# artpixls/ART

Hardware: AMD Instinct MI355X
Metric: megapixels/sec end-to-end (AMaZE+FTblockDN+tone), 45 MP Bayer (higher is better)
Workload: dtype f32; 1 GPU; AMaZE + getImage/matrix + ImProcFunctions::denoise (chroma noise-curve map, FTblockDN wavelet shrinkage luma 40 / chroma 15 / gamma 1.7 + DCT detail recovery 50) + exposure 0.3 EV + tone curve STD, 8192x5464 Bayer RGGB fp32, 1 frame per GPU per step (BASELINE configs[2]); frame=8192x5464, lanes_per_gpu=1, parallelism=frame-per-gpu x1, completion_records=1, completion_via=single process

## Files before the change

### art_amd/csrc/amaze_stream_core.h

```cpp
#pragma once

#ifdef AMZ_EMUL
#include <math.h>
#include <stdint.h>
#include <string.h>
#define AMZ_DEV static inline
typedef float *amz_lf;
typedef unsigned char *amz_lb;
typedef int *amz_li;
typedef unsigned short *amz_ls;
typedef char *amz_lc;
typedef const float *amz_gcf;
typedef float *amz_gf;
namespace amz {
static inline unsigned fc(unsigned filters, unsigned row, unsigned col) { return (filters >> (((((row) << 1) & 14u) + ((col) & 1u)) << 1)) & 3u; }
static inline float sse_min(float x, float y) { return x < y ? x : y; }
static inline float sse_max(float x, float y) { return x > y ? x : y; }
static inline float sqr(float x) { return x * x; }
static inline float intp(float a, float b, float c) { return a * b + (1.f - a) * c; }
static inline float median3(float a, float b, float c) { return sse_max(sse_min(a, b), sse_min(c, sse_max(a, b))); }
static inline float xdiv2f(float d) { int32_t i; memcpy(&i, &d, 4); if (i & 0x7FFFFFFF) i -= 1 << 23; memcpy(&d, &i, 4); return d; }
static inline float xdivf(float d, int n) { int32_t i; memcpy(&i, &d, 4); if (i & 0x7FFFFFFF) i -= n << 23; memcpy(&d, &i, 4); return d; }
static inline int ngroups(int start, int bound, int step) { return bound > start ? (bound - start + step - 1) / step : 0; }
static inline int imin(int a, int b) { return a < b ? a : b; }
// ... 298 lines not shown
        const float cl1 = cr[c - 1], cl2 = cr[c - 2], cr1 = cr[c + 1], cr2 = cr[c + 2];
        const float d0c = d0r[c], d1c = d1r[c];
        const float d0u2 = ROWR(D0, r - 2)[c], d0d2 = ROWR(D0, r + 2)[c], d1l2 = d1r[c - 2], d1r2 = d1r[c + 2];
        const float cru = cu1 * (d0u2 + d0c) / (d0u2 * (eps + cfav) + d0c * (eps + cu2));
        const float crd = cd1 * (d0d2 + d0c) / (d0d2 * (eps + cfav) + d0c * (eps + cd2));
        const float crl = cl1 * (d1l2 + d1c) / (d1l2 * (eps + cfav) + d1c * (eps + cl2));
        const float crr = cr1 * (d1r2 + d1c) / (d1r2 * (eps + cfav) + d1c * (eps + cr2));
        const float guha = cu1 + 0.5f * (cfav - cu2);
        const float gdha = cd1 + 0.5f * (cfav - cd2);
        const float glha = cl1 + 0.5f * (cfav - cl2);
        const float grha = cr1 + 0.5f * (cfav - cr2);
        float guar = fabsf(1.f - cru) < arthresh ? cfav * cru : guha;
        float gdar = fabsf(1.f - crd) < arthresh ? cfav * crd : gdha;
        float glar = fabsf(1.f - crl) < arthresh ? cfav * crl : glha;
        float grar = fabsf(1.f - crr) < arthresh ? cfav * crr : grha;
        const float d1l = d1r[c - 1], d1rr = d1r[c + 1], d0u = ROWR(D0, r - 1)[c], d0d = ROWR(D0, r + 1)[c];
        const float hwt = d1l / (d1l + d1rr);
        const float vwt = d0u / (d0d + d0u);
        const float Ginthha = intp(hwt, grha, glha);
        const float Gintvha = intp(vwt, gdha, guha);
        o_hcdalt = sgn * (Ginthha - cfav);
        o_vcdalt = sgn * (Gintvha - cfav);
        const bool clip = (cfav > a.clip_pt8) || (Gintvha > a.clip_pt8) || (Ginthha > a.clip_pt8);
        if (clip) { guar = guha; gdar = gdha; glar = glha; grar = grha; }
        o_vcd = clip ? o_vcdalt : sgn * (intp(vwt, gdar, guar) - cfav);
        o_hcd = clip ? o_hcdalt : sgn * (intp(hwt, grar, glar) - cfav);
        ROWW(DGV, r)[c] = sse_min(sqr(guha - gdha), sqr(guar - gdar));
        ROWW(DGH, r)[c] = sse_min(sqr(glha - grha), sqr(glar - grar));
        if (!is_green(a, r, c)) {
            amz_lf hv = ROWW(HVW, r);
            hv[c >> 1] = hwt;
            hv[TSH + (c >> 1)] = vwt;
        }
    }
    ROWW(HCA, r)[c] = o_hcdalt;
    ROWW(VCA, r)[c] = o_vcdalt;
    ROWW(VCD, r)[c] = o_vcd;
    ROWW(HCO, r)[c] = o_hcd;
}

AMZ_DEV float p3_hcd_pure(amz_lf ho, amz_lf ha, amz_lf cf, const TileArgs &a, int r, int c)
{
    const float sgn = is_green(a, r, c) ? -1.f : 1.f;
    float hcdv = ho[c];
    const float hv = var3(ho[c - 2], hcdv, ho[c + 2]);
    const float a0 = ha[c];
    const float hav = var3(ha[c - 2], a0, ha[c + 2]);
    hcdv = hav < hv ? a0 : hcdv;
    return bound_cd(hcdv, sgn, cf[c], cf[c - 1], cf[c + 1], a.clip_pt);
}
#ifdef AMZ_EMUL
#define AMZ_P3_COL(c) (c)
#else
#define AMZ_P3_COL(c) ((c) - 2)
#endif
AMZ_DEV void st_p3(amz_lf lds, const TileArgs &a, int r, int c_in)
{
    const int c = AMZ_P3_COL(c_in);
#ifdef AMZ_EMUL
    if (r < 4 || r >= a.rr1 - 4 || c >= TS) return;
#else
    if (r < 4 || r >= a.rr1 - 4) return;
#endif
    float nh = 0.f;
    const bool dom = c >= 4 && c < TS - 4;
    amz_lf ho = ROWR(HCO, r), ha = ROWR(HCA, r), cf = ROWR(CFA, r);
    const int idx = c - 4, k = idx & 3, g = idx >> 2;
#ifndef AMZ_EMUL
    float pure = 0.f;
    if (dom) pure = p3_hcd_pure(ho, ha, cf, a, r, c);
    const float left2 = __shfl_up(pure, 2);
    if (c < 0 || c >= TS) return;
#endif
    if (dom) {
        if (k >= 2) {
#ifdef AMZ_EMUL
            nh = p3_hcd_pure(ho, ha, cf, a, r, c);
#else
            nh = pure;
#endif
        } else {
#ifdef AMZ_EMUL
            const float hm2 = g > 0 ? p3_hcd_pure(ho, ha, cf, a, r, c - 2) : ho[c - 2];
#else
            const float hm2 = g > 0 ? left2 : ho[c - 2];
#endif
            const float sgn = is_green(a, r, c) ? -1.f : 1.f;
            float hcdv = ho[c];
            const float hv = var3(hm2, hcdv, ho[c + 2]);
            const float a0 = ha[c];
            const float hav = var3(ha[c - 2], a0, ha[c + 2]);
            hcdv = hav < hv ? a0 : hcdv;
            nh = bound_cd(hcdv, sgn, cf[c], cf[c - 1], cf[c + 1], a.clip_pt);
        }
        const float sgn = is_green(a, r, c) ? -1.f : 1.f;
        amz_lf vr = ROWR(VCD, r);
        const float n2 = ROWR(VCD, r - 2)[c];
        const float o0 = vr[c], o2 = ROWR(VCD, r + 2)[c];
        const float am2 = ROWR(VCA, r - 2)[c], a0 = ROWR(VCA, r)[c], a2 = ROWR(VCA, r + 2)[c];
        const float cm1 = ROWR(CFA, r - 1)[c], c0 = cf[c], cp1 = ROWR(CFA, r + 1)[c];
        float vcdv = o0;
        const float vv = var3(n2, vcdv, o2);
        const float vav = var3(am2, a0, a2);
        vcdv = vav < vv ? a0 : vcdv;
        const float nv = bound_cd(vcdv, sgn, c0, cm1, cp1, a.clip_pt);
        vr[c] = nv;
        const float cdq = sqr(nv - nh);
        ROWW(CDD, r)[c] = cdq;
        if (r == 19 && c >= 80 && c < 120) lds[NQA_OFF + (c - 80)] = cdq;
    }
    ROWW(HCN, r)[c] = nh;
}

AMZ_DEV int site_sel(const TileArgs &a, int r, int c) { return (c ^ row_par(a, r)) & 1; }

AMZ_DEV void st_p4(amz_lf lds, const TileArgs &a, int r, int c)
{
    if (c >= TS) return;
    const int sl = site_sel(a, r, c), rr = r + sl;
    if (rr < 6 || rr >= a.rr1 - 6) return;
    const int par = row_par(a, rr);
    if (c < 6 + par || c > 156 + par) return;
    amz_lf hn = SROWR(HCN, r, 0, sl), dh = SROWR(DGH, r, 0, sl);
    float tv = SROWR(VCD, r, 0, sl)[c];
    const float vu1 = SROWR(VCD, r, -1, sl)[c], vu2 = SROWR(VCD, r, -2, sl)[c], vu3 = SROWR(VCD, r, -3, sl)[c];
    const float vd1 = SROWR(VCD, r, +1, sl)[c], vd2 = SROWR(VCD, r, +2, sl)[c], vd3 = SROWR(VCD, r, +3, sl)[c];
    const float uave = tv + vu1 + vu2 + vu3;
    const float dave = tv + vd1 + vd2 + vd3;
    float Dvu = sqr(tv - uave) + sqr(vu1 - uave) + sqr(vu2 - uave) + sqr(vu3 - uave);
    float Dvd = sqr(tv - dave) + sqr(vd1 - dave) + sqr(vd2 - dave) + sqr(vd3 - dave);
    amz_lf hv = SROWR(HVW, r, 0, sl);
    const float hwt = hv[c >> 1], vwt = hv[TSH + (c >> 1)];
    const float vcd_c = tv;
    tv = hn[c];
#define COLZ(row, cc) ((cc) < TS ? (row)[cc] : 0.f)
    const float hl1 = hn[c - 1], hl2 = hn[c - 2], hl3 = hn[c - 3];
    const float hr1 = COLZ(hn, c + 1), hr2 = COLZ(hn, c + 2), hr3 = COLZ(hn, c + 3);
    const float lave = tv + (hl3 + hl2) + hl1;
    const float rave = tv + (hr1 + hr2) + hr3;
    float Dhl = sqr(tv - lave) + sqr(hl1 - lave) + sqr(hl2 - lave) + sqr(hl3 - lave);
    float Dhr = sqr(tv - rave) + sqr(hr1 - rave) + sqr(hr2 - rave) + sqr(hr3 - rave);
    const float vcdvar = epssq + intp(vwt, Dvd, Dvu);
    const float hcdvar = epssq + intp(hwt, Dhr, Dhl);
    Dvu = SROWR(DGV, r, -1, sl)[c] + SROWR(DGV, r, -2, sl)[c];
    Dvd = SROWR(DGV, r, +1, sl)[c] + SROWR(DGV, r, +2, sl)[c];
    Dhl = dh[c - 2] + dh[c - 1];
    Dhr = COLZ(dh, c + 1) + COLZ(dh, c + 2);
#undef COLZ
    const float vcdvar1 = epssq + SROWR(DGV, r, 0, sl)[c] + intp(vwt, Dvd, Dvu);
    const float hcdvar1 = epssq + dh[c] + intp(hwt, Dhr, Dhl);
    const float varwt = hcdvar / (vcdvar + hcdvar);
    const float diffwt = hcdvar1 / (vcdvar1 + hcdvar1);
    const bool dec = ((0.5f - varwt) * (0.5f - diffwt) > 0.f) && (fabsf(0.5f - diffwt) < fabsf(0.5f - varwt));
    SROWW(HVWT, r, 0, sl)[c >> 1] = dec ? varwt : diffwt;
    amz_lf vh = SROWW(VH, r, 0, sl);
    vh[c >> 1] = vcd_c;
    vh[TSH + (c >> 1)] = tv;
}

struct ThreadRegs { int bb[4]; int pos_p, pos_h, pos_stride2, pos_off4; };
AMZ_DEV void bb_reset(int *bb) { bb[0] = 1 << 30; bb[1] = 0; bb[2] = 1 << 30; bb[3] = 0; }
AMZ_DEV void bb_add(int *bb, int rr, int cc) { bb[0] = imin(bb[0], rr); bb[1] = imax(bb[1], rr); bb[2] = imin(bb[2], cc); bb[3] = imax(bb[3], cc); }
AMZ_DEV void bb_flush(amz_lf lds, int base, const int *bb)
{
    if (bb[1] == 0 && bb[3] == 0) return;
    amz_li red = (amz_li)(lds + RED_OFF) + base;
#ifdef AMZ_EMUL
    red[0] = imin(red[0], bb[0]); red[1] = imax(red[1], bb[1]); red[2] = imin(red[2], bb[2]); red[3] = imax(red[3], bb[3]);
#else
    __hip_atomic_fetch_min(&red[0], bb[0], __ATOMIC_RELAXED, __HIP_MEMORY_SCOPE_WORKGROUP);
    __hip_atomic_fetch_max(&red[1], bb[1], __ATOMIC_RELAXED, __HIP_MEMORY_SCOPE_WORKGROUP);
    __hip_atomic_fetch_min(&red[2], bb[2], __ATOMIC_RELAXED, __HIP_MEMORY_SCOPE_WORKGROUP);
    __hip_atomic_fetch_max(&red[3], bb[3], __ATOMIC_RELAXED, __HIP_MEMORY_SCOPE_WORKGROUP);
#endif
}

AMZ_DEV void pos_init(amz_lf lds, int c, ThreadRegs &rg)
{
    if (c >= POS_PAIRS) return;
    rg.pos_h = POSTAB.h[c]; rg.pos_stride2 = POSTAB.stride2[c]; rg.pos_off4 = POSTAB.off4[c];
    rg.pos_p = (rg.pos_h - POSTAB.j[c]) % rg.pos_h;
    ((amz_li)(lds + POS_OFF))[c] = rg.pos_off4 + rg.pos_p * rg.pos_stride2;
}
AMZ_DEV void pos_produce(amz_lf lds, int T, int c, ThreadRegs &rg)
{
    if (c >= POS_PAIRS) return;
    rg.pos_p = rg.pos_p + 1 == rg.pos_h ? 0 : rg.pos_p + 1;
    ((amz_li)(lds + POS_OFF + ((T + 1) & 1) * POS_PAIRS))[c] = rg.pos_off4 + rg.pos_p * rg.pos_stride2;
}

AMZ_DEV void st_p5(amz_lf lds, const TileArgs &a, int r, int c, ThreadRegs &rg)
{
    if (r + 1 < 6 || r >= a.rr1 - 6) return;
    if (c >= TS) {
        const int h = c - TS;
        if (h < 12) {
            const int sl = h >= 6, k = h % 6;
            if (r + sl < 6 || r + sl >= a.rr1 - 6) return;
            amz_lb nb = (amz_lb)SROWW(NYQ, r, 0, sl);
            nb[k < 3 ? k : 74 + k] = 0;
        }
        return;
    }
    const int sl = site_sel(a, r, c), rr = r + sl;
    if (rr < 6 || rr >= a.rr1 - 6) return;
    const int par = row_par(a, rr);
    if (c < 6 + par) return;
    amz_lb nb = (amz_lb)SROWW(NYQ, r, 0, sl);
    if (c >= TS - 6) { nb[c >> 1] = 0; return; }
    const float go0 = 0.14659727707323927f, go1 = 0.103592713382435f, go2 = 0.0732036125103057f, go3 = 0.0365543548389495f;
    const float nyqthresh = 0.5f;
    const float gg0 = nyqthresh * 0.07384411893421103f, gg1 = nyqthresh * 0.06207511968171489f, gg2 = nyqthresh * 0.0521818194747806f;
    const float gg3 = nyqthresh * 0.03687419286733595f, gg4 = nyqthresh * 0.03099732204057846f, gg5 = nyqthresh * 0.018413194161458882f;
    const int si = (c - 6 - par) >> 1;
    const bool vec = si < 4 * ngroups(6 + par, TS - 7, 8);
    amz_lf c0 = SROWR(CDD, r, 0, sl), cu1 = SROWR(CDD, r, -1, sl), cu2 = SROWR(CDD, r, -2, sl), cd1 = SROWR(CDD, r, +1, sl), cd2 = SROWR(CDD, r, +2, sl);
    amz_lf d0 = SROWR(DHV, r, 0, sl), du1 = SROWR(DHV, r, -1, sl), du2 = SROWR(DHV, r, -2, sl), dd1 = SROWR(DHV, r, +1, sl), dd2 = SROWR(DHV, r, +2, sl);
    const float gA = go0 * c0[c] +
                     go1 * (cu1[c - 1] + cu1[c + 1] + cd1[c - 1] + cd1[c + 1]) +
                     go2 * (cu2[c] + c0[c - 2] + c0[c + 2] + cd2[c]) +
                     go3 * (cu2[c - 2] + cu2[c + 2] + cd2[c - 2] + cd2[c + 2]);
    const float s1 = vec ? (du1[c] + d0[c - 1] + d0[c + 1] + dd1[c])
                         : (du1[c] + d0[c + 1] + d0[c - 1] + dd1[c]);
    const float gB = gg0 * d0[c] + gg1 * s1 +
                     gg2 * (du1[c - 1] + du1[c + 1] + dd1[c - 1] + dd1[c + 1]) +
                     gg3 * (du2[c] + d0[c - 2] + d0[c + 2] + dd2[c]) +
                     gg4 * (du2[c - 1] + du2[c + 1] + du1[c - 2] + du1[c + 2] +
                            dd1[c - 2] + dd1[c + 2] + dd2[c - 1] + dd2[c + 1]) +
                     gg5 * (du2[c - 2] + du2[c + 2] + dd2[c - 2] + dd2[c + 2]);
    const bool flag = gA - gB > 0.f;
    nb[c >> 1] = flag ? 1 : 0;
    if (flag) bb_add(rg.bb, rr, c);
}

AMZ_DEV void st_p7(amz_lf lds, const TileArgs &a, int r, int item)
{
    if (item >= 2 * TSH) return;
    const int sl = item >= TSH, rr = r + sl, b = item - (sl ? TSH : 0);
    if (rr < 2 || rr >= a.rr1 - 2) return;
    amz_lb out = (amz_lb)SROWW(NYQ2, r, 0, sl);
    if (rr < ny_r0(a) || rr >= ny_r1(a)) {
        out[b] = rr >= TS - 4 ? ((amz_lb)(lds + NQA_OFF))[(rr - (TS - 4)) * TSH + b] : 0;
        return;
    }
    amz_lb n0 = (amz_lb)SROWR(NYQ, r, 0, sl), nu1 = (amz_lb)SROWR(NYQ, r, -1, sl), nu2 = (amz_lb)SROWR(NYQ, r, -2, sl);
    amz_lb nd1 = (amz_lb)SROWR(NYQ, r, +1, sl), nd2 = (amz_lb)SROWR(NYQ, r, +2, sl);
    const int bl = b - 1, br = b + 1;
    const int t = (int)nu2[b] + (bl >= 0 ? (int)nu1[bl] : 0) + (int)nu1[b] + (bl >= 0 ? (int)n0[bl] : 0) +
                  (br < TSH ? (int)n0[br] : 0) + (bl >= 0 ? (int)nd1[bl] : 0) + (int)nd1[b] + (int)nd2[b];
    unsigned char val = n0[b];
    if (t > 4) val = 1;
    if (t < 4) val = 0;
    out[b] = val;
}

AMZ_DEV bool nyq_site(amz_lf lds, const TileArgs &a, int r, int c, int *prr)
{
    if (c >= TS) return false;
    const int sl = site_sel(a, r, c), rr = r + sl;
    *prr = rr;
    if (rr < ny_r0(a) || rr >= ny_r1(a) || c < ny_c0(a) + row_par(a, rr) || c >= ny_c1(a)) return false;
    return ((amz_lb)SROWR(NYQ2, r, 0, sl))[c >> 1] != 0;
}

struct P8Acc { float sumcfa, sumh, sumv, sumsqh, sumsqv, areawt; };
template <int A0, int A1>
AMZ_DEV void p8_accumulate(amz_lf lds, const TileArgs &a, int r, int sl, int cc, P8Acc &s)
{
    const int idx0 = (cc - 6) >> 1;
#pragma unroll
    for (int ai = A0; ai <= A1; ai += 2) {
        amz_lb nq = (amz_lb)SROWR(NYQ2, r, ai, sl);
        amz_lf cr = SROWR(CFA, r, ai, sl), cu = SROWR(CFA, r, ai - 1, sl), cd = SROWR(CFA, r, ai + 1, sl);
#pragma unroll
        for (int bj = 0; bj < 7; ++bj) {
            const bool f = nq[idx0 + bj] != 0;
            const int col = cc - 6 + 2 * bj;
            const float ct = cr[col], cl = cr[col - 1], cq = cr[col + 1], cn = cu[col], cs = cd[col];
            const float t1 = f ? ct : 0.f;
            const float t2 = f ? (cl + cq) : 0.f;
            const float t3 = f ? (cn + cs) : 0.f;
            const float t4 = f ? (sqr(ct - cl) + sqr(ct - cq)) : 0.f;
            const float t5 = f ? (sqr(ct - cn) + sqr(ct - cs)) : 0.f;
            s.sumcfa += t1;
            s.sumh += t2;
            s.sumv += t3;
            s.sumsqh += t4;
            s.sumsqv += t5;
            s.areawt += f ? 1.f : 0.f;
        }
    }
}
AMZ_DEV void p8_finish(amz_lf lds, const TileArgs &a, int r, int sl, int cc, const P8Acc &s, int *bb)
{
    const int rr = r + sl;
    const float sumh = s.sumcfa - xdiv2f(s.sumh);
    const float sumv = s.sumcfa - xdiv2f(s.sumv);
    const float areawt = xdiv2f(s.areawt);
    const float hcdvar = epssq + fabsf(areawt * s.sumsqh - sumh * sumh);
    const float vcdvar = epssq + fabsf(areawt * s.sumsqv - sumv * sumv);
    SROWR(HVWT, r, 0, sl)[cc >> 1] = hcdvar / (vcdvar + hcdvar);
    bb_add(bb, rr, cc);
}
struct P8Regs { P8Acc acc; int sl, cc; };
AMZ_DEV void p8_wave_a(amz_lf lds, const TileArgs &a, int t, int r, int lane, P8Regs &pr)
{
    amz_li red = (amz_li)(lds + RED_OFF);
    amz_ls list = (amz_ls)(lds + LIST_OFF + (t & 1) * LIST_INTS);
    const int n = red[16 + (t & 1)];
    pr.cc = -1;
    if (lane < n) {
        const int e = list[lane];
        pr.sl = (e >> 8) - r; pr.cc = e & 255;
        pr.acc = P8Acc{0.f, 0.f, 0.f, 0.f, 0.f, 0.f};
        p8_accumulate<-6, 0>(lds, a, r, pr.sl, pr.cc, pr.acc);
    }
}
AMZ_DEV void p8_wave_b(amz_lf lds, const TileArgs &a, int t, int r, int lane, P8Regs &pr, int *bb)
{
    amz_li red = (amz_li)(lds + RED_OFF);
    amz_ls list = (amz_ls)(lds + LIST_OFF + (t & 1) * LIST_INTS);
    const int n = red[16 + (t & 1)];
    if (pr.cc >= 0) {
        p8_accumulate<2, 6>(lds, a, r, pr.sl, pr.cc, pr.acc);
        p8_finish(lds, a, r, pr.sl, pr.cc, pr.acc, bb);
    }
    for (int q = 64 + lane; q < n; q += 64) {
        const int e = list[q];
        const int sl = (e >> 8) - r, cc = e & 255;
        P8Acc acc{0.f, 0.f, 0.f, 0.f, 0.f, 0.f};
        p8_accumulate<-6, 0>(lds, a, r, sl, cc, acc);
        p8_accumulate<2, 6>(lds, a, r, sl, cc, acc);
        p8_finish(lds, a, r, sl, cc, acc, bb);
    }
}

AMZ_DEV float p9_new_weight(amz_lf lds, const TileArgs &a, int rr, int j)
{
    const int cc = 8 + row_par(a, rr) + 2 * j;
    amz_lf hu = ROWR(HVWT, rr - 1), hd = ROWR(HVWT, rr + 1);
    const float hvwtalt = xdivf(hu[(cc - 1) >> 1] + hu[(cc + 1) >> 1] + hd[(cc - 1) >> 1] + hd[(cc + 1) >> 1], 2);
    const float h0 = ROWR(HVWT, rr)[cc >> 1];
    return fabsf(0.5f - h0) < fabsf(0.5f - hvwtalt) ? hvwtalt : h0;
}
AMZ_DEV void p9_site(amz_lf lds, const TileArgs &a, int rr, int j, float h)
{
    const int cc = 8 + row_par(a, rr) + 2 * j, idx = cc >> 1;
    ROWR(HVWT, rr)[idx] = h;
    amz_lf vh = ROWR(VH, rr), cr = ROWR(CFA, rr);
    const float dg = intp(h, vh[idx], vh[TSH + idx]);
    ROWW(DG0, rr)[idx] = dg;
    const float gval = cr[cc] + dg;
    ROWW(RGBG, rr)[idx] = gval;
    const bool ny = ((amz_lb)ROWR(NYQ2, rr))[idx] != 0;
    amz_lf d2 = ROWW(DG2, rr);
    d2[2 * idx] = ny ? sqr(gval - xdiv2f(cr[cc - 1] + cr[cc + 1])) : 0.f;
    d2[2 * idx + 1] = ny ? sqr(gval - xdiv2f(ROWR(CFA, rr - 1)[cc] + ROWR(CFA, rr + 1)[cc])) : 0.f;
}

AMZ_DEV void st_p11(amz_lf lds, const TileArgs &a, int r, int item)
{
    if (item >= 152) return;
    const int sl = item >= 76, rr = r + sl, j = item - (sl ? 76 : 0);
    if (rr < 6 || rr >= a.rr1 - 6) return;
    const int e = 6 + 2 * j, idx = e >> 1;
    const bool rbEven = row_par(a, rr) == 0;
    const int g = rbEven ? e + 1 : e;
    const int q = rbEven ? e : e + 1;
    amz_lf cr = SROWR(CFA, r, 0, sl), cu = SROWR(CFA, r, -1, sl), cd = SROWR(CFA, r, +1, sl);
    const float t = cr[g];
    const float sp = sqr(t - cd[g - 1]) + sqr(t - cu[g + 1]);
    const float sm = sqr(t - cu[g - 1]) + sqr(t - cd[g + 1]);
    SROWW(DELP, r, 0, sl)[idx] = fabsf(cu[q + 1] - cd[q - 1]);
    SROWW(DELM, r, 0, sl)[idx] = fabsf(cd[q + 1] - cu[q - 1]);
    SROWW(DM, r, 0, sl)[idx] = sm;
    SROWW(DP, r, 0, sl)[idx] = sp;
}

AMZ_DEV void st_p12(amz_lf lds, const TileArgs &a, int r, int c)
{
    if (r + 1 < 8 || r >= a.rr1 - 8) return;
    if (c >= TS) {
        const int h = c - TS;
        if (h < 8) {
            const int sl = h >= 4, rr = r + sl, k = h & 3;
            if (rr < 8 || rr >= a.rr1 - 8) return;
            SROWW(PMWT, r, 0, sl)[76 + k] = lds[SIDE_OFF + ((rr >> 1) - 4) * 8 + (rr & 1) * 4 + k];
        }
        return;
    }
    const int sl = site_sel(a, r, c), rr = r + sl;
    if (rr < 8 || rr >= a.rr1 - 8) return;
    const int par = row_par(a, rr);
    if (c < 8 + par || c > 150 + par) return;
    const int idx = c >> 1;
    const float ge0 = 0.13719494435797422f, ge1 = 0.05640252782101291f;
    amz_lf c0 = SROWR(CFA, r, 0, sl), cu1 = SROWR(CFA, r, -1, sl), cu2 = SROWR(CFA, r, -2, sl), cd1 = SROWR(CFA, r, +1, sl), cd2 = SROWR(CFA, r, +2, sl);
    const float cfav = c0[c];
    const float cse = cd1[c + 1], cnw = cu1[c - 1], cne = cu1[c + 1], csw = cd1[c - 1];
    const float rbse = rb_ratio(cfav, cse, cd2[c + 2]);
    const float rbnw = rb_ratio(cfav, cnw, cu2[c - 2]);
    amz_lf dm0 = SROWR(DELM, r, 0, sl), dmu1 = SROWR(DELM, r, -1, sl), dmu2 = SROWR(DELM, r, -2, sl), dmd1 = SROWR(DELM, r, +1, sl), dmd2 = SROWR(DELM, r, +2, sl);
    float t1 = eps + dm0[idx];
    const float wtse = t1 + dmd1[(c + 1) >> 1] + dmd2[(c + 2) >> 1];
    const float wtnw = t1 + dmu1[(c - 1) >> 1] + dmu2[(c - 2) >> 1];
    const float rbmv = (wtse * rbnw + wtnw * rbse) / (wtse + wtnw);
    const float rbm_out = rb_bound(rbmv, cfav, cnw, cse, a.clip_pt);
    const float rbne = rb_ratio(cfav, cne, cu2[c + 2]);
    const float rbsw = rb_ratio(cfav, csw, cd2[c - 2]);
    amz_lf dp0 = SROWR(DELP, r, 0, sl), dpu1 = SROWR(DELP, r, -1, sl), dpu2 = SROWR(DELP, r, -2, sl), dpd1 = SROWR(DELP, r, +1, sl), dpd2 = SROWR(DELP, r, +2, sl);
    t1 = eps + dp0[idx];
    const float wtne = t1 + dpu1[(c + 1) >> 1] + dpu2[(c + 2) >> 1];
    const float wtsw = t1 + dpd1[(c - 1) >> 1] + dpd2[(c - 2) >> 1];
    const float rbpv = (wtne * rbsw + wtsw * rbne) / (wtne + wtsw);
    const float rbp_out = rb_bound(rbpv, cfav, csw, cne, a.clip_pt);
    amz_lf m0 = SROWR(DM, r, 0, sl), mu1 = SROWR(DM, r, -1, sl), mu2 = SROWR(DM, r, -2, sl), md1 = SROWR(DM, r, +1, sl), md2 = SROWR(DM, r, +2, sl);
    amz_lf q0 = SROWR(DP, r, 0, sl), qu1 = SROWR(DP, r, -1, sl), qu2 = SROWR(DP, r, -2, sl), qd1 = SROWR(DP, r, +1, sl), qd2 = SROWR(DP, r, +2, sl);
    const float rbvarm = epssq + (ge0 * (mu1[c >> 1] + m0[(c - 1) >> 1] + m0[(c + 1) >> 1] + md1[c >> 1]) +
                                  ge1 * (mu2[(c - 1) >> 1] + mu2[(c + 1) >> 1] + mu1[(c - 2) >> 1] + mu1[(c + 2) >> 1] +
                                         md1[(c - 2) >> 1] + md1[(c + 2) >> 1] + md2[(c - 1) >> 1] + md2[(c + 1) >> 1]));
    const float rbvarp = epssq + (ge0 * (qu1[c >> 1] + q0[(c - 1) >> 1] + q0[(c + 1) >> 1] + qd1[c >> 1]) +
                                  ge1 * (qu2[(c - 1) >> 1] + qu2[(c + 1) >> 1] + qu1[(c - 2) >> 1] + qu1[(c + 2) >> 1] +
                                         qd1[(c - 2) >> 1] + qd1[(c + 2) >> 1] + qd2[(c - 1) >> 1] + qd2[(c + 1) >> 1]));
    SROWW(RBM, r, 0, sl)[idx] = rbm_out;
    SROWW(RBP, r, 0, sl)[idx] = rbp_out;
    SROWW(PMWT, r, 0, sl)[idx] = rbvarm / (rbvarp + rbvarm);
}

AMZ_DEV float p13_new_weight(amz_lf lds, const TileArgs &a, int rr, int j)
{
    const int cc = 10 + row_par(a, rr) + 2 * j;
    amz_lf pu = ROWR(PMWT, rr - 1), pd = ROWR(PMWT, rr + 1);
    const float alt = 0.25f * (pu[(cc - 1) >> 1] + pu[(cc + 1) >> 1] + pd[(cc - 1) >> 1] + pd[(cc + 1) >> 1]);
    const float t = ROWR(PMWT, rr)[cc >> 1];
    return fabsf(0.5f - t) < fabsf(0.5f - alt) ? alt : t;
}
AMZ_DEV void p13_site(amz_lf lds, const TileArgs &a, int rr, int j, float nt)
{
    const int cc = 10 + row_par(a, rr) + 2 * j, idx = cc >> 1;
    ROWR(PMWT, rr)[idx] = nt;
    ROWW(RBINT, rr)[idx] = 0.5f * (ROWR(CFA, rr)[cc] + intp(nt, ROWX(RBP, rr)[idx], ROWX(RBM, rr)[idx]));
}

AMZ_DEV float dirwt_v(amz_lf cm2, amz_lf cm1, amz_lf c0r, amz_lf cp1, amz_lf cp2, int c)
{
    const float c0 = c0r[c];
    const float delv = fabsf(cp1[c] - cm1[c]);
    return eps + fabsf(cp2[c] - c0) + fabsf(c0 - cm2[c]) + delv;
}
AMZ_DEV float dirwt_h(amz_lf cr, int c)
{
    const float c0 = cr[c];
    const float delh = fabsf(cr[c + 1] - cr[c - 1]);
    return eps + fabsf(cr[c + 2] - c0) + fabsf(c0 - cr[c - 2]) + delh;
}

AMZ_DEV void p15_store(amz_lf lds, const TileArgs &a, int r, int sl, int c, bool in14, float dg, float gval)
{
    const int rr = r + sl, idx = c >> 1;
    SROWR(RGBG, r, 0, sl)[idx] = gval;
    if (in14 && (rr & 1) != a.ey) {
        SROWW(DG1, r, 0, sl)[idx] = dg;
        SROWR(DG0, r, 0, sl)[idx] = 0.f;
    } else {
        SROWR(DG0, r, 0, sl)[idx] = dg;
    }
}
AMZ_DEV bool p14_in_range(const TileArgs &a, int rr, int c) { const int par = row_par(a, rr); return rr >= 12 && rr < a.rr1 - 12 && c >= 12 + par && c <= 146 + par; }
AMZ_DEV int st_p1014_classify(amz_lf lds, const TileArgs &a, int r, int c, int *entry)
{
    *entry = 0;
    if (c >= TS) return 0;
    const int sl = site_sel(a, r, c), rr = r + sl;
    *entry = (sl << 8) | c;
    if (rr < 8 || rr >= a.rr1 - 8) return 0;
    const int par = row_par(a, rr), idx = c >> 1;
    if (c < 8 + par || c >= TS - 8) return 0;
    const bool in14 = p14_in_range(a, rr, c);
    if (in14 && fabsf(0.5f - SROWR(PMWT, r, 0, sl)[idx]) >= fabsf(0.5f - SROWR(HVWT, r, 0, sl)[idx])) return 2;
    if (rr >= ny_r0(a) && rr < ny_r1(a) && c >= ny_c0(a) + par && c < ny_c1(a) && ((amz_lb)SROWR(NYQ2, r, 0, sl))[idx]) return 1;
    p15_store(lds, a, r, sl, c, in14, SROWR(DG0, r, 0, sl)[idx], SROWR(RGBG, r, 0, sl)[idx]);
    return 0;
}
AMZ_DEV void p10_site(amz_lf lds, const TileArgs &a, int r, int sl, int c)
{
    const int idx = c >> 1;
    const float gq0 = 0.169917f, gq1 = 0.108947f, gq2 = 0.069855f, gq3 = 0.0287182f;
    amz_lf e0 = SROWX(DG2, r, 0, sl), eu1 = SROWX(DG2, r, -1, sl), eu2 = SROWX(DG2, r, -2, sl), ed1 = SROWX(DG2, r, +1, sl), ed2 = SROWX(DG2, r, +2, sl);
#define DH(row, col) (row)[(col) & ~1]
#define DV(row, col) (row)[(col) | 1]
    const float gvarh = epssq + (gq0 * DH(e0, c) +
                                 gq1 * (DH(eu1, c - 1) + DH(eu1, c + 1) + DH(ed1, c - 1) + DH(ed1, c + 1)) +
                                 gq2 * (DH(eu2, c) + DH(e0, c - 2) + DH(e0, c + 2) + DH(ed2, c)) +
                                 gq3 * (DH(eu2, c - 2) + DH(eu2, c + 2) + DH(ed2, c - 2) + DH(ed2, c + 2)));
    const float gvarv = epssq + (gq0 * DV(e0, c) +
                                 gq1 * (DV(eu1, c - 1) + DV(eu1, c + 1) + DV(ed1, c - 1) + DV(ed1, c + 1)) +
                                 gq2 * (DV(eu2, c) + DV(e0, c - 2) + DV(e0, c + 2) + DV(ed2, c)) +
                                 gq3 * (DV(eu2, c - 2) + DV(eu2, c + 2) + DV(ed2, c - 2) + DV(ed2, c + 2)));
#undef DH
#undef DV
    amz_lf vh = SROWR(VH, r, 0, sl);
    const float dg = (vh[TSH + idx] * gvarv + vh[idx] * gvarh) / (gvarv + gvarh);
    p15_store(lds, a, r, sl, c, p14_in_range(a, r + sl, c), dg, SROWR(CFA, r, 0, sl)[c] + dg);
}
AMZ_DEV void p14_site(amz_lf lds, const TileArgs &a, int r, int sl, int c)
{
    const int idx = c >> 1;
    const float hw = SROWR(HVWT, r, 0, sl)[idx];
    amz_lf rb0 = SROWR(RBINT, r, 0, sl);
    const float rb = rb0[idx];
    amz_lf f3u = SROWR(CFA, r, -3, sl), f2u = SROWR(CFA, r, -2, sl), f1u = SROWR(CFA, r, -1, sl), f0 = SROWR(CFA, r, 0, sl);
    amz_lf f1d = SROWR(CFA, r, +1, sl), f2d = SROWR(CFA, r, +2, sl), f3d = SROWR(CFA, r, +3, sl);
    const float cfav = f0[c];
    const float cu = f1u[c], cd = f1d[c], cl = f0[c - 1], cr = f0[c + 1];
    const float gu = g_dir(rb, cu, SROWR(RBINT, r, -2, sl)[idx]);
    const float gd = g_dir(rb, cd, SROWR(RBINT, r, +2, sl)[idx]);
    const float d0u = dirwt_v(f3u, f2u, f1u, f0, f1d, c), d0d = dirwt_v(f1u, f0, f1d, f2d, f3d, c);
    float Gintv = (d0u * gd + d0d * gu) / (d0d + d0u);
    Gintv = g_bound(Gintv, rb, cu, cd, a.clip_pt);
    const float gl = g_dir(rb, cl, rb0[idx - 1]);
    const float gr = g_dir(rb, cr, rb0[idx + 1]);
    const float d1l = dirwt_h(f0, c - 1), d1r = dirwt_h(f0, c + 1);
    float Ginth = (d1l * gr + d1r * gl) / (d1l + d1r);
    Ginth = g_bound(Ginth, rb, cl, cr, a.clip_pt);
    const float gval = intp(hw, Gintv, Ginth);
    p15_store(lds, a, r, sl, c, true, gval - cfav, gval);
}
AMZ_DEV void hot_append(amz_lf lds, int which, bool flag, int entry)
{
    amz_li hot = (amz_li)(lds + HOT_OFF);
#ifdef AMZ_EMUL
    if (flag) hot[2 + which * 160 + hot[which]++] = entry;
#else
    const unsigned long long m = __ballot(flag);
    if (m) {
        const int lane = (int)(threadIdx.x & 63u);
        int base = 0;
        if (lane == 0) base = __hip_atomic_fetch_add(&hot[which], __popcll(m), __ATOMIC_RELAXED, __HIP_MEMORY_SCOPE_WORKGROUP);
        base = __builtin_amdgcn_readfirstlane(base);
        if (flag) hot[2 + which * 160 + base + __popcll(m & ((1ull << lane) - 1ull))] = entry;
    }
#endif
}
AMZ_DEV void st_p1014_light(amz_lf lds, const TileArgs &a, int r, int c)
{
    int entry;
    const int kind = st_p1014_classify(lds, a, r, c, &entry);
    hot_append(lds, 0, kind == 1, entry);
    hot_append(lds, 1, kind == 2, entry);
}
AMZ_DEV void p10_worker(amz_lf lds, const TileArgs &a, int r, int lane)
{
    amz_li hot = (amz_li)(lds + HOT_OFF);
    const int n = hot[0];
    for (int q = lane; q < n; q += 64) { const int e = hot[2 + q]; p10_site(lds, a, r, e >> 8, e & 255); }
}
AMZ_DEV void p14_worker(amz_lf lds, const TileArgs &a, int r, int lane)
{
    amz_li hot = (amz_li)(lds + HOT_OFF);
    const int n = hot[1];
    for (int q = lane; q < n; q += 64) { const int e = hot[2 + 160 + q]; p14_site(lds, a, r, e >> 8, e & 255); }
}
AMZ_DEV void hot_reset(amz_lf lds, int which) { ((amz_li)(lds + HOT_OFF))[which] = 0; }

AMZ_DEV void st_p16(amz_lf lds, const TileArgs &a, int r, int c)
{
    if (c >= TS) return;
    const int sl = site_sel(a, r, c), rr = r + sl;
    if (rr < 14 || rr >= a.rr1 - 14) return;
    const int par = row_par(a, rr);
    if (c < 14 + par || c > 148 + par) return;
    const bool red_row = (rr & 1) == a.ey;
#define DROW(k) (red_row ? SROWX(DG1, r, (k), sl) : SROWX(DG0, r, (k), sl))
    amz_lf u1 = DROW(-1), u3 = DROW(-3), d1 = DROW(1), d3 = DROW(3);
#undef DROW
#define AT(row, col) (row)[(col) >> 1]
    const float dnw = AT(u1, c - 1), dse = AT(d1, c + 1), dne = AT(u1, c + 1), dsw = AT(d1, c - 1);
    const float dnw3 = AT(u3, c - 3), dse3 = AT(d3, c + 3), dne3 = AT(u3, c + 3), dsw3 = AT(d3, c - 3);
    const float temp = eps + fabsf(dnw - dse);
    const float temp2 = eps + fabsf(dne - dsw);
    const float wtnw = 1.f / (temp + fabsf(dnw - dnw3) + fabsf(dse - dnw3));
    const float wtne = 1.f / (temp2 + fabsf(dne - dne3) + fabsf(dsw - dne3));
    const float wtsw = 1.f / (temp2 + fabsf(dsw - dse3) + fabsf(dne - dsw3));
    const float wtse = 1.f / (temp + fabsf(dse - dsw3) + fabsf(dnw - dse3));
    const float val = (wtnw * (1.325f * dnw - 0.175f * dnw3 - 0.075f * (AT(u1, c - 3) + AT(u3, c - 1))) +
                       wtne * (1.325f * dne - 0.175f * dne3 - 0.075f * (AT(u1, c + 3) + AT(d1, c + 1))) +
                       wtsw * (1.325f * dsw - 0.175f * dsw3 - 0.075f * (AT(d1, c - 3) + AT(u1, c - 1))) +
                       wtse * (1.325f * dse - 0.175f * dse3 - 0.075f * (AT(d1, c + 3) + AT(d3, c + 1)))) /
                      (wtnw + wtne + wtsw + wtse);
#undef AT
    if (red_row) SROWW(DG1, r, 0, sl)[c >> 1] = val; else SROWR(DG0, r, 0, sl)[c >> 1] = val;
}

AMZ_DEV void st_out(amz_lf lds, const TileArgs &a, int rr, int c)
{
    if (rr < 16 || rr >= a.rr1 - 16 || c < 16 || c >= TS - 16) return;
    float gval, rv, bv;
    if (is_green(a, rr, c)) {
        gval = ROWR(CFA, rr)[c];
        amz_lf hu = ROWR(HVWT, rr - 1), h0 = ROWR(HVWT, rr), hd = ROWR(HVWT, rr + 1);
        const float h_up = hu[c >> 1], h_dn = hd[c >> 1], h_r = h0[(c + 1) >> 1], h_l = h0[(c - 1) >> 1];
        const float temp = 1.f / (h_up + 2.f - h_r - h_l + h_dn);
        amz_lf a0u = ROWR(DG0, rr - 1), a00 = ROWR(DG0, rr), a0d = ROWR(DG0, rr + 1);
        amz_lf a1u = ROWR(DG1, rr - 1), a10 = ROWR(DG1, rr), a1d = ROWR(DG1, rr + 1);
        rv = gval - (h_up * a0u[c >> 1] + (1.f - h_r) * a00[(c + 1) >> 1] + (1.f - h_l) * a00[(c - 1) >> 1] + h_dn * a0d[c >> 1]) * temp;
        bv = gval - (h_up * a1u[c >> 1] + (1.f - h_r) * a10[(c + 1) >> 1] + (1.f - h_l) * a10[(c - 1) >> 1] + h_dn * a1d[c >> 1]) * temp;
    } else {
        gval = ROWR(RGBG, rr)[c >> 1];
        rv = gval - ROWR(DG0, rr)[c >> 1];
        bv = gval - ROWR(DG1, rr)[c >> 1];
    }
    const long o = (long)(rr + a.top) * a.os + (a.left + c);
    a.red[o] = sse_max(65535.f * rv, 0.f);
    a.blue[o] = sse_max(65535.f * bv, 0.f);
    a.green[o] = sse_max(gval * 65535.f, 0.f);
}



AMZ_DEV bool tile_valid(amz_lf lds, int par, int rr1, int *box)
{
    amz_li red = (amz_li)(lds + RED_OFF) + 8 * par;
    int nystartrow = red[0] == (1 << 30) ? 0 : red[0], nyendrow = red[1], nystartcol = red[2], nyendcol = red[3];
    const bool doNyquist = nystartrow != nyendrow && nystartcol != nyendcol;
    if (doNyquist) {
        nyendrow++;
        nyendcol++;
        nystartcol -= (nystartcol & 1);
        nystartrow = imax(8, nystartrow);
        nyendrow = imin(rr1 - 8, nyendrow);
        nystartcol = imax(8, nystartcol);
        nyendcol = imin(TS - 8, nyendcol);
    } else {
        nystartrow = nyendrow = nystartcol = nyendcol = 0;
    }
    box[0] = nystartrow; box[1] = nyendrow; box[2] = nystartcol; box[3] = nyendcol;
// ... 174 lines not shown
```

Before: 4612 MP/s.

## Split sparse AMaZE pass-8 sites across lane pairs with DPP partner reduction

When the per-row list of Nyquist sites is small (at most 32), each site is now handled by two adjacent lanes. Each lane of the pair accumulates half of the window terms, and the halves are combined with a DPP row-shuffle, so more of the wavefront does useful work. The count is read once with readfirstlane and carried in registers, and the overflow loop for larger lists is restructured to reuse the wave_a/wave_b accumulator path. The risks are extra DPP instructions, divergence on the odd lanes, and an out-of-range read by the odd lane, which is guarded by a static_assert.

```diff
diff --git a/art_amd/csrc/amaze_stream_core.h b/art_amd/csrc/amaze_stream_core.h
--- a/art_amd/csrc/amaze_stream_core.h
+++ b/art_amd/csrc/amaze_stream_core.h
@@ -624,36 +624,111 @@
     SROWR(HVWT, r, 0, sl)[cc >> 1] = hcdvar / (vcdvar + hcdvar);
     bb_add(bb, rr, cc);
 }
-struct P8Regs { P8Acc acc; int sl, cc; };
+#if !defined(AMZ_EMUL) || defined(AMZ_P8_PAIR_HOST)
+#ifdef AMZ_P8_PAIR_HOST
+float p8_partner(float v);
+#else
+AMZ_DEV float p8_partner(float v)
+{
+    return __builtin_bit_cast(float, __builtin_amdgcn_update_dpp(0, __builtin_bit_cast(int, v), 0xF5, 0xf, 0xf, true));
+}
+#endif
+template <int A0, int A1>
+AMZ_DEV void p8_accumulate_pair(amz_lf lds, const TileArgs &a, int r, int sl, int cc, int odd, P8Acc &s)
+{
+    static_assert(CFA_OFF + CFA_D * CFA_S + 3 <= LDS_FLOATS && NYQ2_OFF + NYQ2_D * NYQ2_S + 1 <= LDS_FLOATS, "the odd lane's unused fourth term reads inside LDS");
+    const int idx0 = ((cc - 6) >> 1) + odd, col0 = cc - 6 + 2 * odd;
+#pragma unroll
+    for (int ai = A0; ai <= A1; ai += 2) {
+        amz_lb nq = (amz_lb)SROWR(NYQ2, r, ai, sl);
+        amz_lf cr = SROWR(CFA, r, ai, sl), cu = SROWR(CFA, r, ai - 1, sl), cd = SROWR(CFA, r, ai + 1, sl);
+#pragma unroll
+        for (int k = 0; k < 4; ++k) {
+            const bool f = nq[idx0 + 2 * k] != 0;
+            const int col = col0 + 4 * k;
+            const float ct = cr[col], cl = cr[col - 1], cq = cr[col + 1], cn = cu[col], cs = cd[col];
+            const float x2 = cl + cq, x3 = cn + cs, x4 = sqr(ct - cl) + sqr(ct - cq), x5 = sqr(ct - cn) + sqr(ct - cs);
+            const float t1 = f ? ct : 0.f, t2 = f ? x2 : 0.f, t3 = f ? x3 : 0.f, t4 = f ? x4 : 0.f, t5 = f ? x5 : 0.f, t6 = f ? 1.f : 0.f;
+            s.sumcfa += t1;
+            s.sumh += t2;
+            s.sumv += t3;
+            s.sumsqh += t4;
+            s.sumsqv += t5;
+            s.areawt += t6;
+            if (k == 3) break;
+            s.sumcfa += p8_partner(t1);
+            s.sumh += p8_partner(t2);
+            s.sumv += p8_partner(t3);
+            s.sumsqh += p8_partner(t4);
+            s.sumsqv += p8_partner(t5);
+            s.areawt += p8_partner(t6);
+        }
+    }
+}
+#endif
+constexpr int P8_PAIR_MAX = 32;
+#ifdef AMZ_P8_COUNT
+static long long g_p8_count[146];
+#endif
+struct P8Regs { P8Acc acc; int sl, cc, n; };
 AMZ_DEV void p8_wave_a(amz_lf lds, const TileArgs &a, int t, int r, int lane, P8Regs &pr)
 {
     amz_li red = (amz_li)(lds + RED_OFF);
     amz_ls list = (amz_ls)(lds + LIST_OFF + (t & 1) * LIST_INTS);
-    const int n = red[16 + (t & 1)];
+#ifndef AMZ_EMUL
+    int nv = red[16 + (t & 1)], e1 = list[lane], e2 = list[lane >> 1];
+    asm volatile("" : "+v"(nv), "+v"(e1), "+v"(e2));
+    const int n = __builtin_amdgcn_readfirstlane(nv);
+#else
+    const int n = red[16 + (t & 1)], e1 = list[lane];
+#endif
     pr.cc = -1;
+    pr.n = n;
+#ifdef AMZ_P8_COUNT
+    if (lane == 0) g_p8_count[n < 145 ? n : 145]++;
+#endif
+#ifndef AMZ_EMUL
+    if (n <= P8_PAIR_MAX) {
+        if (lane < 2 * n) {
+            pr.sl = (e2 >> 8) - r; pr.cc = e2 & 255;
+            pr.acc = P8Acc{0.f, 0.f, 0.f, 0.f, 0.f, 0.f};
+            p8_accumulate_pair<-6, 0>(lds, a, r, pr.sl, pr.cc, lane & 1, pr.acc);
+        }
+        return;
+    }
+#endif
     if (lane < n) {
-        const int e = list[lane];
-        pr.sl = (e >> 8) - r; pr.cc = e & 255;
+        pr.sl = (e1 >> 8) - r; pr.cc = e1 & 255;
         pr.acc = P8Acc{0.f, 0.f, 0.f, 0.f, 0.f, 0.f};
         p8_accumulate<-6, 0>(lds, a, r, pr.sl, pr.cc, pr.acc);
     }
 }
 AMZ_DEV void p8_wave_b(amz_lf lds, const TileArgs &a, int t, int r, int lane, P8Regs &pr, int *bb)
 {
-    amz_li red = (amz_li)(lds + RED_OFF);
     amz_ls list = (amz_ls)(lds + LIST_OFF + (t & 1) * LIST_INTS);
-    const int n = red[16 + (t & 1)];
-    if (pr.cc >= 0) {
-        p8_accumulate<2, 6>(lds, a, r, pr.sl, pr.cc, pr.acc);
-        p8_finish(lds, a, r, pr.sl, pr.cc, pr.acc, bb);
-    }
-    for (int q = 64 + lane; q < n; q += 64) {
-        const int e = list[q];
-        const int sl = (e >> 8) - r, cc = e & 255;
-        P8Acc acc{0.f, 0.f, 0.f, 0.f, 0.f, 0.f};
-        p8_accumulate<-6, 0>(lds, a, r, sl, cc, acc);
-        p8_accumulate<2, 6>(lds, a, r, sl, cc, acc);
-        p8_finish(lds, a, r, sl, cc, acc, bb);
+    const int n = pr.n;
+#ifndef AMZ_EMUL
+    if (n <= P8_PAIR_MAX) {
+        if (pr.cc >= 0) {
+            p8_accumulate_pair<2, 6>(lds, a, r, pr.sl, pr.cc, lane & 1, pr.acc);
+            if (!(lane & 1)) p8_finish(lds, a, r, pr.sl, pr.cc, pr.acc, bb);
+        }
+        return;
+    }
+#endif
+    for (int q0 = 64;; q0 += 64) {
+        if (pr.cc >= 0) {
+            p8_accumulate<2, 6>(lds, a, r, pr.sl, pr.cc, pr.acc);
+            p8_finish(lds, a, r, pr.sl, pr.cc, pr.acc, bb);
+        }
+        if (q0 >= n) break;
+        pr.cc = -1;
+        if (q0 + lane < n) {
+            const int e = list[q0 + lane];
+            pr.sl = (e >> 8) - r; pr.cc = e & 255;
+            pr.acc = P8Acc{0.f, 0.f, 0.f, 0.f, 0.f, 0.f};
+            p8_accumulate<-6, 0>(lds, a, r, pr.sl, pr.cc, pr.acc);
+        }
     }
 }
 
```

Result: no change. 4646 MP/s, median of 6 (+0.7%).
